# folkol/query-engines

Hardware: AMD Instinct MI355X
Metric: rows/sec filter+project+group-by over 1B-row Arrow batch; % HBM roofline (higher is better)
Workload: dtype int64; 1 GPU; C4: SELECT k, SUM(a+b), COUNT(*), MIN(a), MAX(b) WHERE a > 2^19 GROUP BY k; rows_per_gpu=1000000000, groups=1024, columns=k, a, b int64 (Arrow, no nulls), parallelism=hash-sharded partial aggregate x1

## Files before the change

### query-engines_amd/csrc/qe_jit.hip

```cpp
#include <hip/hiprtc.h>
#include <stdio.h>
#include <stdlib.h>
#include <fcntl.h>
#include <string.h>
#include <sys/stat.h>
#include <unistd.h>

#include <map>
#include <mutex>
#include <sstream>
#include <vector>

#include "qe_internal.hpp"

namespace qe {

static const char* kDevHeader =
#include "qe_dev.inc"
    ;

namespace {

struct Expr {
  std::string v;
  std::string ok;
  bool f;
};

std::string col_raw(int c) { return "c" + std::to_string(c) + "[r]"; }
std::string col_ok(const Plan& P, int c) {
  return P.cols[c].valid ? "((v" + std::to_string(c) + " >> r) & 1u)" : std::string("1u");
}
bool col_is_f(const Plan& P, int c) { return P.cols[c].kind == K_F64; }
std::string col_val(const Plan& P, int c) {
  return col_is_f(P, c) ? "bits_f64(" + col_raw(c) + ")" : col_raw(c);
}

bool agg_expr(const Plan& P, int j, Expr* out) {
  const DAgg& a = P.aggs[j];
  std::vector<Expr> st;
  for (int t = 0; t < a.ntok; ++t) {
    const DTok& k = a.tok[t];
    const std::string litref = "P.aggs[" + std::to_string(j) + "].tok[" + std::to_string(t) + "].lit";
    switch (k.op) {
      case T_COL: st.push_back({col_val(P, k.arg), col_ok(P, k.arg), col_is_f(P, k.arg)}); break;
      case T_LIT:
        st.push_back({k.lit_f64 ? "bits_f64(" + litref + ")" : litref, k.lit_null ? "0u" : "1u", k.lit_f64 != 0});
        break;
      case T_I2F0:
        if (st.empty()) return false;
        st.back() = {"((double)(" + st.back().v + "))", st.back().ok, true};
        break;
      case T_I2F1:
        if (st.size() < 2) return false;
        st[st.size() - 2] = {"((double)(" + st[st.size() - 2].v + "))", st[st.size() - 2].ok, true};
        break;
      default: {
        if (st.size() < 2) return false;
        const Expr b = st.back();
        st.pop_back();
        const Expr l = st.back();
        st.pop_back();
        Expr e;
        e.ok = "(" + l.ok + " & " + b.ok + ")";
        switch (k.op) {
          case T_ADD_I: e = {"((qi64)((qu64)(" + l.v + ") + (qu64)(" + b.v + ")))", e.ok, false}; break;
          case T_SUB_I: e = {"((qi64)((qu64)(" + l.v + ") - (qu64)(" + b.v + ")))", e.ok, false}; break;
          case T_MUL_I: e = {"((qi64)((qu64)(" + l.v + ") * (qu64)(" + b.v + ")))", e.ok, false}; break;
          case T_DIV_I:
            e = {"idiv((" + l.v + "), (" + b.v + "))", "(" + e.ok + " & (qu32)((" + b.v + ") != 0))", false};
            break;
          case T_ADD_F: e = {"((" + l.v + ") + (" + b.v + "))", e.ok, true}; break;
          case T_SUB_F: e = {"((" + l.v + ") - (" + b.v + "))", e.ok, true}; break;
          case T_MUL_F: e = {"((" + l.v + ") * (" + b.v + "))", e.ok, true}; break;
          case T_DIV_F: e = {"((" + l.v + ") / (" + b.v + "))", e.ok, true}; break;
          default: return false;
        }
        st.push_back(e);
      }
    }
  }
  if (st.size() != 1) return false;
  *out = st[0];
  if (out->f) out->v = "f64_bits(" + out->v + ")";
  return true;
}

const char* cmp_sym(int op) {
  switch (op) {
    case QE_OP_EQ: return "==";
    case QE_OP_NE: return "!=";
    case QE_OP_LT: return "<";
    case QE_OP_LE: return "<=";
    case QE_OP_GT: return ">";
    default: return ">=";
  }
}

std::string acc_init(int acc) {
  switch (acc) {
    case ACC_MIN_I:
    case ACC_MIN_F: return "0x7FFFFFFFFFFFFFFFll";
    case ACC_MAX_I:
    case ACC_MAX_F: return "EMPTY_KEY";
    default: return "0";
  }
}

bool use_nt() {
  const char* e = getenv("QE_NT");
  return !(e && e[0] == '0');
}
}

bool fused_prefetch() {
  static const bool v = [] {
    const char* e = getenv("QE_FUSED_PF");
    return e && e[0] == '1';
  }();
  return v;
}
int fused_block(int lds_log2) {
  (void)lds_log2;
  static const int env = [] {
    const char* e = getenv("QE_FUSED_BLOCK");
    const int b = e ? atoi(e) : 0;
    return (b == 256 || b == 512 || b == 1024) ? b : 0;
  }();
  return env ? env : 1024;
}

namespace {

std::string ld(const std::string& type, const std::string& ptr, bool nt = true) {
  if (nt && use_nt()) return "__builtin_nontemporal_load((const " + type + "*)(" + ptr + "))";
  return "(*(const " + type + "*)(" + ptr + "))";
}

void emit_predicate(const Plan& P, std::ostringstream& o, int rows) {
  const std::string loop = "#pragma unroll\n    for (int r = 0; r < " + std::to_string(rows) + "; ++r) ";
  if (P.mask_col >= 0) {
    o << loop << "if (!((qu32)(" << col_raw(P.mask_col) << " & 1) & " << col_ok(P, P.mask_col)
      << ")) act &= ~(1u << r);\n";
  }
  for (int t = 0; t < P.nterms; ++t) {
    const DTerm& T = P.terms[t];
    const std::string lit = "P.terms[" + std::to_string(t) + "].lit";
    std::string lhs, rhs, ok = col_ok(P, T.lhs);
    if (T.f64) {
      lhs = col_is_f(P, T.lhs) ? col_val(P, T.lhs) : "((double)" + col_raw(T.lhs) + ")";
      if (T.rhs >= 0) rhs = col_is_f(P, T.rhs) ? col_val(P, T.rhs) : "((double)" + col_raw(T.rhs) + ")";
      else rhs = "bits_f64(" + lit + ")";
    } else {
      lhs = col_raw(T.lhs);
      rhs = T.rhs >= 0 ? col_raw(T.rhs) : lit;
    }
    if (T.rhs >= 0) ok += " & " + col_ok(P, T.rhs);
    else if (T.lit_null) ok = "0u";
    o << loop << "if (!((" << lhs << ") " << cmp_sym(T.op) << " (" << rhs << ")) || !(" << ok
      << ")) act &= ~(1u << r);\n";
  }
}

unsigned pred_key_cols(const Plan& P) {
  unsigned m = 0;
  if (P.mask_col >= 0) m |= 1u << P.mask_col;
  for (int t = 0; t < P.nterms; ++t) {
    m |= 1u << P.terms[t].lhs;
    if (P.terms[t].rhs >= 0) m |= 1u << P.terms[t].rhs;
  }
  if (P.key_mode != 0)
    for (int k = 0; k < P.nkeys; ++k) m |= 1u << P.key_col[k];
  return m;
}

void emit_col_loads(const Plan& P, std::ostringstream& o, unsigned need, const std::string& pre = "c",
                    bool declare = true) {
  const std::string vpre = pre == "c" ? "v" : "p" + std::string("v");
  for (int c = 0; c < P.ncols; ++c) {
    if (!((need >> c) & 1u)) continue;
    const std::string cs = std::to_string(c);
    const std::string dst = pre + cs;
    if (declare) o << "    qi64 " << dst << "[4];\n";
    const int kind = P.cols[c].kind;
    const char* ty = kind == K_I32 ? "qi32" : kind == K_U8 ? "qu8" : kind == K_BOOL ? "qu8" : "qi64";
    o << "    {\n      const " << ty << "* p = (const " << ty << "*)P.cols[" << cs << "].p;\n";
    if (kind == K_BOOL) {
      o << "      for (int r = 0; r < 4; ++r) { const qi64 row = r0 + 128 * (r >> 1) + (r & 1);\n"
        << "        " << dst << "[r] = (full || row < P.n) ? ((p[row >> 3] >> (row & 7)) & 1) : 0; }\n";
    } else {
      o << "      if (full) {\n";
      if (kind == K_I64 || kind == K_F64) {
        o << "        const qi64x2 a = " << ld("qi64x2", "p + r0") << ", b = " << ld("qi64x2", "p + r0 + 128") << ";\n"
          << "        " << dst << "[0] = a.x; " << dst << "[1] = a.y; " << dst << "[2] = b.x; " << dst << "[3] = b.y;\n";
      } else if (kind == K_I32) {
        o << "        const qi32x2 a = " << ld("qi32x2", "p + r0") << ", b = " << ld("qi32x2", "p + r0 + 128") << ";\n"
          << "        " << dst << "[0] = a.x; " << dst << "[1] = a.y; " << dst << "[2] = b.x; " << dst << "[3] = b.y;\n";
      } else {
        o << "        const qu16 a = " << ld("qu16", "p + r0") << ", b = " << ld("qu16", "p + r0 + 128") << ";\n"
          << "        " << dst << "[0] = a & 0xFF; " << dst << "[1] = a >> 8; " << dst << "[2] = b & 0xFF; " << dst
          << "[3] = b >> 8;\n";
      }
      o << "      } else {\n"
        << "        for (int r = 0; r < 4; ++r) { const qi64 row = r0 + 128 * (r >> 1) + (r & 1);\n"
        << "          " << dst << "[r] = row < P.n ? (qi64)p[row] : 0; }\n      }\n";
    }
    o << "    }\n";
    if (P.cols[c].valid) {
      if (declare) o << "    qu32 " << vpre << cs << ";\n";
      o << "    {\n      const qu8* vb = P.cols[" << cs << "].valid;\n"
        << "      const qu32 lo = (full || r0 < P.n) ? ((qu32)(vb[r0 >> 3] >> (r0 & 7)) & 3u) : 0u;\n"
        << "      const qu32 hi = (full || r0 + 128 < P.n) ? ((qu32)(vb[(r0 + 128) >> 3] >> (r0 & 7)) & 3u) : 0u;\n"
        << "      " << vpre << cs << " = lo | (hi << 2);\n    }\n";
    }
  }
}

void emit_active_rows(const Plan& P, std::ostringstream& o, bool retry, bool skip_idle = true) {
  o << "    qu32 act = 15u;\n"
    << "    if (!full) { act = 0; for (int r = 0; r < 4; ++r) act |= (qu32)(r0 + 128 * (r >> 1) + (r & 1) < P.n) << r; }\n";
  if (retry)
    o << "    if (P.defer_in) {\n      for (int r = 0; r < 4; ++r) { const qi64 row = r0 + 128 * (r >> 1) + (r & 1);\n"
      << "        if (row < P.n && !((P.defer_in[row >> 5] >> (row & 31)) & 1)) act &= ~(1u << r); }\n    }\n";
  emit_predicate(P, o, 4);
  if (skip_idle) o << "    if (act == 0) continue;\n";
}

void emit_keys(const Plan& P, std::ostringstream& o) {
  o << "    qi64 key[4] = {0, 0, 0, 0};\n    qu32 knull = 0;\n";
  if (P.key_mode == 1) {
    const int c = P.key_col[0];
    o << "#pragma unroll\n    for (int r = 0; r < 4; ++r) {\n      qi64 k = " << col_raw(c) << ";\n";
    if (P.key_f64) o << "      if (bits_f64(k) != bits_f64(k)) k = 0x7FF8000000000000ll;\n";
    if (P.cols[c].valid)
      o << "      if (!" << col_ok(P, c) << ") { k = 0; knull |= 1u << r; }\n";
    o << "      key[r] = k;\n    }\n";
  } else if (P.key_mode == 2) {
    o << "#pragma unroll\n    for (int r = 0; r < 4; ++r) {\n      qi64 k = 0;\n";
    for (int q = 0; q < P.nkeys; ++q) {
      const int c = P.key_col[q];
      o << "      { const bool isn = !" << col_ok(P, c) << "; k |= ((isn ? 0ll : (" << col_raw(c) << " & "
        << P.key_fmask[q] << "ll)) << " << P.key_shift[q] << ") | ((qi64)isn << " << P.key_nullbit[q] << "); }\n";
    }
    o << "      key[r] = k;\n    }\n";
  }
}

void emit_lds_table(const Plan& P, std::ostringstream& o, int log2, size_t* lds_bytes) {
  const int S = 1 << log2, SS = S + 2;
  o << "  constexpr int LOG2 = " << log2 << ", S = " << S << ", SS = " << SS << ";\n"
    << "  __shared__ qi64 s_keys[SS];\n  __shared__ qu32 s_cst[SS];\n";
  size_t lds = (size_t)SS * 12;
  for (int j = 0; j < P.naggs; ++j) {
    const DAgg& a = P.aggs[j];
    if (a.share) {
      const int i = a.share - 1;
      if (a.acc != ACC_NONE) o << "  qi64* const s_acc" << j << " = s_acc" << i << ";\n";
      if (a.track_nn) o << "  qu32* const s_nn" << j << " = s_nn" << i << ";\n";
      if (acc_has_idx(a.acc)) o << "  qu64* const s_idx" << j << " = s_idx" << i << ";\n";
      continue;
    }
    if (a.acc != ACC_NONE) {
      o << "  __shared__ qi64 s_acc" << j << "[SS];\n";
      lds += 8 * SS;
    }
    if (a.track_nn) {
      o << "  __shared__ qu32 s_nn" << j << "[SS];\n";
      lds += 4 * SS;
    }
    if (acc_has_idx(a.acc)) {
      const int nw = a.acc == ACC_SUM_X ? fx_window_idx_words() : 4;
      o << "  __shared__ qu64 s_idx" << j << "[" << nw << " * SS];\n";
      lds += 8 * nw * SS;
    }
  }
  *lds_bytes = lds;
  o << "  for (int s = threadIdx.x; s < SS; s += blockDim.x) {\n    s_keys[s] = EMPTY_KEY;\n    s_cst[s] = 0;\n";
  for (int j = 0; j < P.naggs; ++j) {
    const DAgg& a = P.aggs[j];
    if (a.share) continue;
    if (a.acc != ACC_NONE) o << "    s_acc" << j << "[s] = " << acc_init(a.acc) << ";\n";
    if (a.track_nn) o << "    s_nn" << j << "[s] = 0;\n";
    if (acc_has_idx(a.acc))
      o << "    for (int k = 0; k < " << (a.acc == ACC_SUM_X ? fx_window_idx_words() : 4) << "; ++k) s_idx" << j << "[k * SS + s] = "
        << (acc_is_f64mm(a.acc) ? "~0ull" : "0ull") << ";\n";
  }
  o << "  }\n  __syncthreads();\n";
}

constexpr int FXQ_CAP = 128;

std::vector<int> fx_queue_aggs(const Plan& P) {
  std::vector<int> q;
  for (int j = 0; j < P.naggs; ++j)
    if (P.aggs[j].pkind != 0 && P.aggs[j].acc == ACC_SUM_X && !P.aggs[j].share) q.push_back(j);
  return q;
}

bool fx_queue_enabled() {
  static const bool v = [] {
    const char* e = getenv("QE_FX_QUEUE");
    return !(e && e[0] == '0');
  }();
  return v;
}

size_t fx_queue_bytes(const Plan& P, int block) {
  const size_t nq = fx_queue_aggs(P).size();
  return nq ? (size_t)(block / 64) * FXQ_CAP * (4 + 8 * nq) : 0;
}

void emit_fx_queue_decl(const Plan& P, std::ostringstream& o, int block) {
  const std::vector<int> q = fx_queue_aggs(P);
  o << "  __shared__ qu32 q_slot[" << (block / 64) * FXQ_CAP << "];\n";
  for (size_t k = 0; k < q.size(); ++k) o << "  __shared__ qi64 q_x" << k << "[" << (block / 64) * FXQ_CAP << "];\n";
  o << "  const qu32 q_base = (threadIdx.x >> 6) * " << FXQ_CAP << "u;\n  qu32 q_head = 0, q_n = 0;\n";
}

void emit_fx_queue_run(const Plan& P, std::ostringstream& o, const std::string& m) {
  const std::vector<int> q = fx_queue_aggs(P);
  const int nq = (int)q.size();
  o << "      __builtin_amdgcn_fence(__ATOMIC_ACQ_REL, \"wavefront\");\n"
    << "      if ((qu32)lane < " << m << ") {\n"
    << "        const qu32 qp = q_base + ((q_head + (qu32)lane) & " << FXQ_CAP - 1 << "u);\n"
    << "        const qu32 qe = q_slot[qp];\n        const int s = (int)(qe & 0xFFFFFFu);\n"
    << "        qi64 qx[" << nq << "];\n        qu32 rare = 0;\n";
  for (int k = 0; k < nq; ++k)
    o << "        qx[" << k << "] = ((qe >> " << 24 + k << ") & 1u) ? q_x" << k << "[qp] : 0ll;\n"
      << "        if (fx_rare(qx[" << k << "])) { rare |= 1u << " << k << "; qx[" << k << "] = 0; }\n";
  {
  o << "        qu64* wp0[" << nq << "];\n        qu64* wp1[" << nq << "];\n        qu64 lo[" << nq << "], hi[" << nq
    << "];\n        bool ng[" << nq << "], k0[" << nq << "];\n";
  for (int k = 0; k < nq; ++k) {
    const std::string j = std::to_string(q[k]), ks = std::to_string(k);
    o << "        {\n          const qu64 b = (qu64)qx[" << ks << "];\n          const int ex = (int)((b >> 52) & 0x7FF);\n"
      << "          const qu64 mm = ex ? ((b & ((1ull << 52) - 1)) | (1ull << 52)) : 0ull;\n"
      << "          const int p = ex ? ex - FXW_EX_LO : 0, kk = p >> 6, qq = p & 63;\n"
      << "          qu64 l = mm << qq, h = qq ? (mm >> (64 - qq)) : 0ull;\n"
      << "          ng[" << ks << "] = ex && (b >> 63);  // (-0.0 adds nothing, like +0.0)\n"
      << "          if (ng[" << ks << "]) { l = 0ull - l; h = ~h + (l == 0 ? 1ull : 0ull); }\n"
      << "          lo[" << ks << "] = l; hi[" << ks << "] = h; k0[" << ks << "] = kk == 0;\n"
      << "          wp0[" << ks << "] = kk ? &s_idx" << j << "[s] : (qu64*)&s_acc" << j << "[s];\n"
      << "          wp1[" << ks << "] = &s_idx" << j << "[kk * SS + s];\n        }\n";
  }
  o << "        qu64 o0[" << nq << "], t[" << nq << "], o1[" << nq << "];\n";
  for (int k = 0; k < nq; ++k) o << "        o0[" << k << "] = atomicAdd(wp0[" << k << "], lo[" << k << "]);\n";
  for (int k = 0; k < nq; ++k)
    o << "        t[" << k << "] = hi[" << k << "] + (o0[" << k << "] + lo[" << k << "] < o0[" << k << "] ? 1ull : 0ull);\n";
  for (int k = 0; k < nq; ++k) o << "        o1[" << k << "] = atomicAdd(wp1[" << k << "], t[" << k << "]);\n";
  for (int k = 0; k < nq; ++k) {
    const std::string j = std::to_string(q[k]), ks = std::to_string(k);
    o << "        if (k0[" << ks << "]) {\n          const qi64 d = (qi64)((t[" << ks << "] < hi[" << ks << "] ? 1 : 0) + (o1[" << ks
      << "] + t[" << ks << "] < o1[" << ks << "] ? 1 : 0)) - (ng[" << ks << "] ? 1 : 0);\n"
      << "          if (d) atomicAdd(&s_idx" << j << "[SS + s], (qu64)d);\n        }\n";
  }
  }
  o << "        if (rare) {\n          const bool knl = s == S;\n"
    << "          const qi64 key = knl ? 0 : (s == S + 1 ? EMPTY_KEY : s_keys[s]);\n";
  for (int k = 0; k < nq; ++k) {
    unsigned jm = 1u << q[k];
// ... 203 lines not shown
    << "      const qu32 kk = (qu32)key[r];\n"
    << "      const int hs = bucket2_hit(q[r], q2[r], kk, h[r], h2[r]);\n"
    << "      slot[r] = ((knull >> r) & 1) ? S : ((qi32)kk == EMPTY_KEY32 ? S + 1 : hs);\n"
    << "    }\n"
    << "    qu32 miss = 0;\n"
    << "#pragma unroll\n    for (int r = 0; r < 4; ++r) miss |= (qu32)(slot[r] < 0) << r;\n"
    << "    miss &= act & fit;\n"
    << "    if (miss) {\n      int t0 = slot[0], t1 = slot[1], t2 = slot[2], t3 = slot[3];\n"
    << "      lds_probe4_rows(s_keys, NBK, miss, (qi32)key[0], (qi32)key[1], (qi32)key[2], (qi32)key[3], h[0], h[1], h[2], h[3], t0, t1, t2, t3);\n"
    << "      slot[0] = t0; slot[1] = t1; slot[2] = t2; slot[3] = t3;\n    }\n"
    << "    qu32 glob = ~fit;\n"
    << "#pragma unroll\n    for (int r = 0; r < 4; ++r) glob |= (qu32)(slot[r] < 0) << r;\n"
    << "    glob &= act;\n    const qu32 loc = act & ~glob;\n"
    << "    int sl[4];\n"
    << "#pragma unroll\n    for (int r = 0; r < 4; ++r) sl[r] = ((loc >> r) & 1) ? slot[r] : SINK + lane;\n"
    << "#pragma unroll\n    for (int r = 0; r < 4; ++r) atomicAdd(&s_cst[sl[r]], 1u);\n";
  for (int j = 0; j < P.naggs; ++j) {
    const DAgg& a = P.aggs[j];
    if (a.pkind == 0) continue;
    const std::string js = std::to_string(j);
    const bool a32 = compact_acc32(P, j);
    o << "#pragma unroll\n    for (int r = 0; r < 4; ++r) {\n"
      << "      const int s = (" << ok[j] << ") ? sl[r] : SINK + lane;\n"
      << "      const qi64 x = " << val[j] << ";\n";
    if (a.track_nn) o << "      atomicAdd(&s_nn" << js << "[s], 1u);\n";
    switch (a.acc) {
      case ACC_SUM_I: o << "      atomicAdd((qu64*)&s_acc" << js << "[s], (qu64)x);\n"; break;
      case ACC_MIN_I: o << "      lds_min_rf(&s_acc" << js << "[s], " << (a32 ? "(qi32)x" : "x") << ");\n"; break;
      case ACC_MAX_I: o << "      lds_max_rf(&s_acc" << js << "[s], " << (a32 ? "(qi32)x" : "x") << ");\n"; break;
      default: break;
    }
    o << "    }\n";
  }
  o << "    if (glob) {\n      for (int r = 0; r < 4; ++r) {\n        if (!((glob >> r) & 1)) continue;\n"
    << "        const qi64 lr = " << didx << ";\n        qu64 gs;\n"
    << "        if (!gtable_find(P.t, key[r], (knull >> r) & 1, gs)) {\n"
    << "          atomicOr((qu32*)&P.defer_out[lr >> 5], 1u << (lr & 31));\n"
    << "          atomicAdd(&P.t.ctl[1], 1ull);\n          continue;\n        }\n"
    << "        gadd_cstar(P.t, gs, 1);\n        const qu64 row = (qu64)(" << row << ");\n";
  for (int j = 0; j < P.naggs; ++j) {
    const DAgg& a = P.aggs[j];
    if (a.pkind == 0) continue;
    o << "        if (" << ok[j] << ") { const RowVal rv = row_partial(" << a.acc << ", " << val[j]
      << ", row); gcombine(P.t, " << a.acc << ", " << j << ", gs, rv.acc, 1, rv.i0, rv.i1, rv.i2, rv.i3, "
      << (((P.nn_skip >> j) & 1) ? "false" : "true") << "); }\n";
  }
  o << "      }\n    }\n";
}

void emit_flush_c(const Plan& P, std::ostringstream& o) {
  o << "  __syncthreads();\n"
    << "  for (int s = threadIdx.x; s < SS; s += blockDim.x) {\n"
    << "    const qu32 c = s_cst[s];\n    if (c == 0) continue;\n"
    << "    const bool knl = s == S;\n    const qi64 key = knl ? 0 : (s == S + 1 ? (qi64)EMPTY_KEY32 : (qi64)s_keys[s]);\n"
    << "    qu64 gs;\n"
    << "    const bool ok = gtable_find_wg(P.t, key, knl, gs, &s_newg);\n"
    << "    qu8* rec = nullptr;\n"
    << "    if (ok) {\n      gadd_cstar(P.t, gs, c);\n    } else {\n"
    << "      const qu64 ri = atomicAdd(&P.t.ctl[2], 1ull);\n"
    << "      if (ri >= P.ovf_cap) { atomicAdd(&P.t.ctl[3], 1ull); continue; }\n"
    << "      rec = P.ovf + ri * (qu64)P.rec_bytes;\n      write_record_head(rec, key, knl, c);\n    }\n";
  int off = 24;
  for (int j = 0; j < P.naggs; ++j) {
    const DAgg& a = P.aggs[j];
    const std::string js = std::to_string(j);
    o << "    {\n      const qi64 acc = " << (a.acc != ACC_NONE ? "(qi64)s_acc" + js + "[s]" : std::string("0")) << ";\n"
      << "      const qu64 nn = " << (a.track_nn ? "s_nn" + js + "[s]" : std::string("c")) << ";\n";
    const bool skip_nn = (P.nn_skip >> j) & 1;
    if (a.fn != QE_AGG_COUNT_STAR && !(a.acc == ACC_NONE && skip_nn))
      o << "      if (ok) gcombine(P.t, " << a.acc << ", " << j << ", gs, acc, nn, ~0ull, ~0ull, ~0ull, ~0ull, "
        << (skip_nn ? "false" : "true") << ");\n";
    o << "      if (!ok) { qu64* f = (qu64*)(rec + " << off << "); f[0] = (qu64)acc; f[1] = nn; }\n    }\n";
    off += agg_rec_bytes(a.acc);
  }
  o << "  }\n";
}

}

bool agg_inputs(const Plan& P, std::vector<Expr>* ex) {
  ex->assign(P.naggs, Expr{"0", "1u", false});
  for (int j = 0; j < P.naggs; ++j)
    if (P.aggs[j].pkind != 0 && !agg_expr(P, j, &(*ex)[j])) return false;
  return true;
}

}

void emit_record_words(const Plan& P, const PartLayout& L, const std::vector<Expr>& ex, const std::string& dst,
                       std::ostringstream& o);
static void emit_fit_check(const PartLayout& L, const std::string& w, std::ostringstream& o);

bool compact_acc32(const Plan& P, int j) {
  const DAgg& a = P.aggs[j];
  if (a.acc != ACC_MIN_I && a.acc != ACC_MAX_I) return false;
  if (a.ntok != 1 || a.tok[0].op != T_COL) return false;
  const int k = P.cols[a.tok[0].arg].kind;
  return k == K_I64 || k == K_I32 || k == K_U8 || k == K_BOOL;
}

bool compact_ok(const Plan& P) {
  if (P.key_f64 || P.key_mode == 0) return false;
  for (int j = 0; j < P.naggs; ++j) {
    const int acc = P.aggs[j].acc;
    if (acc != ACC_NONE && acc != ACC_SUM_I && acc != ACC_MIN_I && acc != ACC_MAX_I) return false;
  }
  return true;
}

size_t compact_slot_bytes(const Plan& P) {
  size_t b = 8;
  for (int j = 0; j < P.naggs; ++j) {
    if (P.aggs[j].acc != ACC_NONE) b += compact_acc32(P, j) ? 4 : 8;
    if (P.aggs[j].track_nn) b += 4;
  }
  return b;
}

bool gen_fused_source(const Plan& P, int log2, std::string* src, size_t* lds_bytes, bool spill) {
  if (log2 < 4 || log2 > 16 || P.ncols < 1 || P.ncols > QE_MAX_COLS) return false;
  if (spill && P.mp_n < 2) return false;
  const bool compact = P.lds_compact > 0;
  if (compact && !compact_ok(P)) return false;
  std::vector<Expr> ex;
  if (!agg_inputs(P, &ex)) return false;
  std::vector<std::string> val(P.naggs), ok(P.naggs);
  for (int j = 0; j < P.naggs; ++j) {
    val[j] = ex[j].v;
    ok[j] = ex[j].ok;
  }
  std::ostringstream o;
  const bool pf = fused_prefetch();
  o << "\nusing namespace qe;\n"
    << "extern \"C\" __global__ void __launch_bounds__(" << fused_block(log2) << ") qe_fused(const Plan P) {\n"
    << "  __shared__ qu32 s_newg;\n  if (threadIdx.x == 0) s_newg = 0;\n";
  const int SB = spill ? P.mp_n - 1 : 0;
  if (spill && (SB & (SB - 1))) return false;
  if (spill)
    o << "  constexpr int SB = " << SB << ";\n  qi64 sp_cid[SB];\n  qu32 sp_fill[SB];\n"
      << "#pragma unroll\n  for (int b = 0; b < SB; ++b) { sp_cid[b] = -1; sp_fill[b] = 0; }\n  qu32 nfit = 0;\n";
  if (compact) emit_lds_table_c(P, o, lds_bytes);
  else emit_lds_table(P, o, log2, lds_bytes);
  const int block = fused_block(log2);
  const bool fxq = !compact && !spill && P.mp_n <= 1 && fx_queue_enabled() && !fx_queue_aggs(P).empty() &&
                   fx_queue_aggs(P).size() <= 8 && (1 << log2) + 2 < (1 << 24) &&
                   *lds_bytes + fx_queue_bytes(P, block) <= (size_t)152 * 1024;
  if (fxq) {
    emit_fx_queue_decl(P, o, block);
    *lds_bytes += fx_queue_bytes(P, block);
  }
  o << "  const int lane = threadIdx.x & 63;\n"
    << "  const qi64 wave = (blockIdx.x * (qi64)blockDim.x + threadIdx.x) >> 6;\n"
    << "  const qi64 stride = (((qi64)gridDim.x * blockDim.x) >> 6) * 256;\n";
  if (pf) {
    o << "  {\n    const qi64 base = wave * 256;\n    const bool full = base + 256 <= P.n;\n"
      << "    const qi64 r0 = base + 2 * lane;\n";
    emit_col_loads(P, o, ~0u, "p", true);
    o << "  for (qi64 base = wave * 256; base < P.n; base += stride) {\n"
      << "    const bool full = base + 256 <= P.n;\n"
      << "    const qi64 r0 = base + 2 * lane;\n";
    for (int c = 0; c < P.ncols; ++c) {
      o << "    qi64 c" << c << "[4] = {p" << c << "[0], p" << c << "[1], p" << c << "[2], p" << c << "[3]};\n";
      if (P.cols[c].valid) o << "    const qu32 v" << c << " = pv" << c << ";\n";
    }
    o << "    if (base + stride < P.n) {\n      const qi64 nb = base + stride;\n"
      << "      const bool full = nb + 256 <= P.n;\n      const qi64 r0 = nb + 2 * lane;\n";
    emit_col_loads(P, o, ~0u, "p", false);
    o << "    }\n    do {\n";
  } else {
    o << "  for (qi64 base = wave * 256; base < P.n; base += stride) {\n"
      << "    const bool full = base + 256 <= P.n;\n"
      << "    const qi64 r0 = base + 2 * lane;\n";
    emit_col_loads(P, o, ~0u);
  }
  emit_active_rows(P, o, true, !fxq && !spill);
  emit_keys(P, o);
  if (spill) {
    const PartLayout L = part_layout(P);
    const int RB = L.bytes();
    const int wb = L.narrow ? 4 : 8;
    std::vector<std::pair<int, int>> pieces;
    for (int q = 0; q < L.words;) {
      const int left = (L.words - q) * wb;
      const int n = (left >= 16 ? 16 : left >= 12 && L.narrow ? 12 : left >= 8 ? 8 : 4) / wb;
      pieces.push_back({q, n});
      q += n;
    }
    auto piece_store = [&](int q, int n) {
      const int bytes = n * wb;
      o << "            {\n";
      if (bytes == 4) {
        o << "              __builtin_amdgcn_raw_buffer_store_b32((qu32)w[" << q << "], cb, off, " << q * wb << ", 0);\n";
      } else {
        const int d = bytes / 4;
        o << "              qu32x" << d << " v;\n";
        for (int i = 0; i < n; ++i)
          if (L.narrow)
            o << "              v[" << i << "] = (qu32)w[" << q + i << "];\n";
          else
            o << "              v[" << 2 * i << "] = (qu32)w[" << q + i << "]; v[" << 2 * i + 1 << "] = (qu32)((qu64)w[" << q + i
              << "] >> 32);\n";
        o << "              __builtin_amdgcn_raw_buffer_store_b" << bytes * 8 << "(v, cb, off, " << q * wb << ", 0);\n";
      }
      o << "            }\n";
    };
    o << "    qu32 sp = 0, sbk[4] = {0, 0, 0, 0};\n"
      << "#pragma unroll\n    for (int r = 0; r < 4; ++r) {\n"
      << "      const qu32 hs = spill_hash((qu64)key[r]);\n"
      << "      if (((act >> r) & 1) && hs >= P.mp_keep) sp |= 1u << r;\n"
      << "      sbk[r] = hs & (qu32)(SB - 1);\n    }\n"
      << "    act &= ~sp;\n"
      << "#pragma unroll\n    for (int b = 0; b < SB; ++b) {\n      qu64 bal[4];\n      qu32 tot = 0;\n"
      << "#pragma unroll\n      for (int r = 0; r < 4; ++r) { bal[r] = __ballot(((sp >> r) & 1u) && sbk[r] == (qu32)b); tot += (qu32)__popcll(bal[r]); }\n"
      << "      const qu32 room = sp_cid[b] >= 0 ? (qu32)PART_CH - sp_fill[b] : 0u;\n"
      << "      if (tot && tot <= room) {\n"
      << "        const __amdgpu_buffer_rsrc_t cb = __builtin_amdgcn_make_buffer_rsrc((void*)(P.part_rec + sp_cid[b] * (PART_CH * "
      << RB << "ll)), (short)0, (int)(PART_CH * " << RB << "), 0x00020000);\n"
      << "        qu32 kb = 0;\n"
      << "#pragma unroll\n        for (int r = 0; r < 4; ++r) {\n"
      << "          if ((bal[r] >> lane) & 1) {\n"
      << "            const qu32 k = __builtin_amdgcn_mbcnt_hi((qu32)(bal[r] >> 32), __builtin_amdgcn_mbcnt_lo((qu32)bal[r], kb));\n"
      << "            const int off = (int)((sp_fill[b] + k) * " << RB << "u);\n"
      << "            qi64 w[" << L.words << "];\n";
    emit_record_words(P, L, ex, "w", o);
    emit_fit_check(L, "w", o);
    for (const auto& pc : pieces) piece_store(pc.first, pc.second);
    o << "          }\n          kb += (qu32)__popcll(bal[r]);\n        }\n"
      << "        sp_fill[b] += tot;\n"
      << "      } else if (tot) {\n"
      << "        const int leader = __ffsll((long long)__ballot(1)) - 1;\n"
      << "        qi64 id = 0;\n"
      << "        if (lane == leader) {\n"
      << "          if (sp_cid[b] >= 0) P.part_chunk[1 + sp_cid[b]] = ((qi64)b << 32) | PART_CH;\n"
      << "          id = (qi64)atomicAdd((qu64*)P.part_chunk, 1ull);\n"
      << "        }\n"
      << "        id = __shfl(id, leader);\n"
      << "        const qi64 nid = (qi64)(((qu64)__builtin_amdgcn_readfirstlane((qu32)((qu64)id >> 32)) << 32) |\n"
      << "                                (qu64)__builtin_amdgcn_readfirstlane((qu32)id));\n"
      << "        qu32 kb = 0;\n"
      << "#pragma unroll\n        for (int r = 0; r < 4; ++r) {\n"
      << "          if ((bal[r] >> lane) & 1) {\n"
      << "            const qu32 k = kb + (qu32)__popcll(bal[r] & ((1ull << lane) - 1));\n"
      << "            const qu64 pos = k < room ? (qu64)sp_cid[b] * PART_CH + sp_fill[b] + k : (qu64)nid * PART_CH + (k - room);\n"
      << "            qi64 w[" << L.words << "];\n";
    emit_record_words(P, L, ex, "w", o);
    emit_fit_check(L, "w", o);
    const char* wt = L.narrow ? "qi32" : "qi64";
    o << "            " << wt << "* const dst = (" << wt << "*)(P.part_rec + pos * " << RB << "ull);\n";
    for (int q = 0; q < L.words; ++q) o << "            dst[" << q << "] = (" << wt << ")w[" << q << "];\n";
    o << "          }\n          kb += (qu32)__popcll(bal[r]);\n        }\n"
      << "        sp_cid[b] = nid;\n        sp_fill[b] = tot - room;\n"
      << "      }\n    }\n"
      << "    if (act == 0) continue;\n";
  } else if (P.mp_n > 1)
    o << "#pragma unroll\n    for (int r = 0; r < 4; ++r)\n"
      << "      if (((act >> r) & 1) && (P.mp_pass < 0 ? spill_hash((qu64)key[r]) < P.mp_keep\n"
      << "                                              : (qu32)__umul64hi(fmix64((qu64)key[r]), (qu64)P.mp_n) != (qu32)P.mp_pass))\n"
      << "        act &= ~(1u << r);\n"
      << "    if (act == 0) continue;\n";
  if (compact)
    emit_agg_rows_c(P, o, val, ok, "P.row_base + r0 + 128 * (r >> 1) + (r & 1)", "r0 + 128 * (r >> 1) + (r & 1)");
  else
    emit_agg_rows(P, o, val, ok, "P.row_base + r0 + 128 * (r >> 1) + (r & 1)", "r0 + 128 * (r >> 1) + (r & 1)", fxq,
                  log2 <= 8);
  o << (pf ? "    } while (0);\n  }\n  }\n" : "  }\n");
  if (fxq) {
    o << "  if (q_n) {\n";
    emit_fx_queue_run(P, o, "q_n");
    o << "  }\n";
  }
  if (spill)
    o << "#pragma unroll\n  for (int b = 0; b < SB; ++b)\n"
      << "    if ((threadIdx.x & 63) == 0 && sp_cid[b] >= 0) P.part_chunk[1 + sp_cid[b]] = ((qi64)b << 32) | (qi64)sp_fill[b];\n"
      << "  if (nfit) atomicOr(&P.t.ctl[7], 1ull);\n";
  if (compact) emit_flush_c(P, o);
  else emit_flush(P, o);
  o << "  __syncthreads();\n  if (threadIdx.x == 0 && s_newg) atomicAdd(&P.t.ctl[0], (qu64)s_newg);\n}\n";
  static const bool fx_inline = [] {
    const char* e = getenv("QE_FX_INLINE");
    return !(e && e[0] == '0');
  }();
  *src = std::string(fx_inline ? "#define QE_FX_INLINE 1\n" : "") + kDevHeader + o.str();
  return true;
}

PartLayout part_layout(const Plan& P) {
  PartLayout L{};
  bool knull = false, vnull = false, cnull = false;
  for (int k = 0; k < P.nkeys; ++k) knull = knull || P.cols[P.key_col[k]].valid != nullptr;
  int nv = 0;
  unsigned cm = 0;
  for (int j = 0; j < P.naggs; ++j) {
    if (P.aggs[j].pkind == 0) continue;
    ++nv;
    vnull = vnull || P.aggs[j].track_nn;
    L.row = L.row || acc_is_f64mm(P.aggs[j].acc);
    for (int t = 0; t < P.aggs[j].ntok; ++t)
      if (P.aggs[j].tok[t].op == T_COL) cm |= 1u << P.aggs[j].tok[t].arg;
  }
  for (int c = 0; c < P.ncols; ++c)
    if ((cm >> c) & 1u) cnull = cnull || P.cols[c].valid != nullptr;
  const int wv = 1 + nv + ((knull || vnull) ? 1 : 0);
  const int wc = 1 + __builtin_popcount(cm) + ((knull || cnull) ? 1 : 0);
  L.colmode = wc < wv;
  int w = 1;
  for (int j = 0; j < P.naggs; ++j) L.val_word[j] = (!L.colmode && P.aggs[j].pkind != 0) ? w++ : -1;
  for (int c = 0; c < QE_MAX_COLS; ++c) L.col_word[c] = (L.colmode && ((cm >> c) & 1u)) ? w++ : -1;
  L.flags_word = (knull || (L.colmode ? cnull : vnull)) ? w++ : -1;
  L.row_word = L.row ? w++ : -1;
  L.words = w;
  if (P.part_narrow && !L.row && !P.key_f64) {
    bool ok = true;
    for (int c = 0; c < P.ncols; ++c)
      if (L.col_word[c] >= 0 && P.cols[c].kind == K_F64) ok = false;
    for (int j = 0; j < P.naggs; ++j)
      if (L.val_word[j] >= 0 && P.aggs[j].acc != ACC_SUM_I && P.aggs[j].acc != ACC_MIN_I && P.aggs[j].acc != ACC_MAX_I)
        ok = false;
    L.narrow = ok;
  }
  return L;
}

static void emit_fit_check(const PartLayout& L, const std::string& w, std::ostringstream& o) {
  if (!L.narrow) return;
  for (int q = 0; q < L.words; ++q)
    o << "      nfit |= (qu32)((qu64)" << w << "[" << q << "] >> 32) ^ (qu32)((qi32)" << w << "[" << q << "] >> 31);\n";
}

static std::string narrow_chunk(const std::string& w, int G, const std::string& q) {
  if (G == 1) return "(qu32)" + w + "[" + q + "]";
  return "((qu64)(qu32)" + w + "[2 * (" + q + ")] | ((qu64)(qu32)" + w + "[2 * (" + q + ") + 1] << 32))";
}

void emit_record_words(const Plan& P, const PartLayout& L, const std::vector<Expr>& ex, const std::string& dst,
                       std::ostringstream& o) {
  o << "      " << dst << "[0] = key[r];\n";
  for (int j = 0; j < P.naggs; ++j)
    if (L.val_word[j] >= 0) o << "      " << dst << "[" << L.val_word[j] << "] = " << ex[j].v << ";\n";
  for (int c = 0; c < P.ncols; ++c)
    if (L.col_word[c] >= 0) o << "      " << dst << "[" << L.col_word[c] << "] = " << col_raw(c) << ";\n";
  if (L.flags_word >= 0) {
    o << "      " << dst << "[" << L.flags_word << "] = (qi64)((knull >> r) & 1)";
    for (int j = 0; j < P.naggs; ++j)
      if (L.val_word[j] >= 0) o << " | ((qi64)((" << ex[j].ok << ") & 1u) << " << (1 + j) << ")";
    for (int c = 0; c < P.ncols; ++c)
      if (L.col_word[c] >= 0 && P.cols[c].valid) o << " | ((qi64)" << col_ok(P, c) << " << " << (1 + c) << ")";
    o << ";\n";
  }
  if (L.row_word >= 0)
    o << "      " << dst << "[" << L.row_word << "] = P.row_base + r0 + 128 * (r >> 1) + (r & 1);\n";
}

bool gen_part_source(const Plan& P, int log2p, bool scatter, std::string* src) {
  if (P.ncols < 1 || P.ncols > QE_MAX_COLS || log2p < 1 || log2p > 13) return false;
  std::vector<Expr> ex;
  if (!agg_inputs(P, &ex)) return false;
  const PartLayout L = part_layout(P);
  unsigned need = pred_key_cols(P);
  if (scatter) need = ~0u;
  std::ostringstream o;
  o << "\nusing namespace qe;\n"
    << "extern \"C\" __global__ void __launch_bounds__(512) " << (scatter ? "qe_pscatter" : "qe_pcount")
    << "(const Plan P) {\n"
    << "  constexpr int LOG2P = " << log2p << ", NP = 1 << LOG2P;\n";
  if (scatter)
    o << "  __shared__ qu64 s_cur[NP];\n"
      << "  for (int b = threadIdx.x; b < NP; b += blockDim.x) s_cur[b] = (qu64)P.part_off[(qi64)b * gridDim.x + blockIdx.x];\n";
  else
    o << "  __shared__ qu32 s_cnt[NP];\n"
      << "  for (int b = threadIdx.x; b < NP; b += blockDim.x) s_cnt[b] = 0;\n";
  o << "  __syncthreads();\n"
    << "  const int lane = threadIdx.x & 63;\n"
    << "  qu32 nfit = 0;\n"
    << "  const qi64 lo = (qi64)blockIdx.x * P.part_tw;\n"
    << "  const qi64 hi = lo + P.part_tw < P.n ? lo + P.part_tw : P.n;\n"
    << "  for (qi64 base = lo + (qi64)(threadIdx.x >> 6) * 256; base < hi; base += (qi64)(blockDim.x >> 6) * 256) {\n"
    << "    const bool full = base + 256 <= P.n;\n"
    << "    const qi64 r0 = base + 2 * lane;\n";
  emit_col_loads(P, o, need);
  emit_active_rows(P, o, false);
  emit_keys(P, o);
  o << "#pragma unroll\n    for (int r = 0; r < 4; ++r) {\n"
    << "      if (!((act >> r) & 1)) continue;\n"
    << "      const qu32 b = (qu32)(fmix64((qu64)key[r]) >> (64 - LOG2P));\n";
  if (!scatter) {
    o << "      atomicAdd(&s_cnt[b], 1u);\n    }\n  }\n  __syncthreads();\n"
      << "  for (int b = threadIdx.x; b < NP; b += blockDim.x) P.part_off[(qi64)b * gridDim.x + blockIdx.x] = s_cnt[b];\n}\n";
  } else {
    o << "      const qu64 pos = atomicAdd(&s_cur[b], 1ull);\n"
      << "      qi64 w[" << L.words << "];\n";
    emit_record_words(P, L, ex, "w", o);
    emit_fit_check(L, "w", o);
    if (L.narrow) {
      const int G = L.words % 2 ? 1 : 2;
      const char* ct = G == 2 ? "qu64" : "qu32";
      o << "      " << ct << "* dst = (" << ct << "*)(P.part_rec + pos * " << L.bytes() << "ull);\n";
      for (int q = 0; q < L.words / G; ++q)
        o << "      dst[" << q << "] = " << narrow_chunk("w", G, std::to_string(q)) << ";\n";
    } else if (L.words % 2 == 0) {
      o << "      qi64x2* dst = (qi64x2*)(P.part_rec + pos * " << 8 * L.words << "ull);\n";
      for (int q = 0; q < L.words / 2; ++q)
        o << "      dst[" << q << "] = qi64x2{w[" << 2 * q << "], w[" << 2 * q + 1 << "]};\n";
    } else {
      o << "      qi64* dst = (qi64*)(P.part_rec + pos * " << 8 * L.words << "ull);\n";
      for (int q = 0; q < L.words; ++q) o << "      dst[" << q << "] = w[" << q << "];\n";
    }
    o << "    }\n  }\n";
    if (L.narrow) o << "  if (nfit) atomicOr(&P.t.ctl[7], 1ull);\n";
    o << "}\n";
  }
  *src = std::string(kDevHeader) + o.str();
  return true;
}

bool part_staged_ok(const Plan& P, int log2p) {
  if (P.n < 2) return false;
  if (log2p == 10) return pscatter_wide() && part_layout(P).words <= 3;
  return log2p <= 9 && part_layout(P).words * pscatter_block() <= 8 * 256;
// ... 1669 lines not shown
```

Measured before the change: 285.3 billion rows/s.

## Split main scan loop into full-tile and tail paths with compile-time full flag

Restructures the JIT-emitted scan loop so full 256-row tiles run in a loop where `full` is a constexpr true, and the partial tail runs once afterwards. This removes per-iteration bounds checks and branches in the hot path. The prefetch path is rewritten to match. It also adds environment-gated experiment modes (QE_EXP) that insert s_waitcnt barriers or unroll two tiles per iteration. These modes are probes and are off by default.

```diff
diff --git a/query-engines_amd/csrc/qe_jit.hip b/query-engines_amd/csrc/qe_jit.hip
--- a/query-engines_amd/csrc/qe_jit.hip
+++ b/query-engines_amd/csrc/qe_jit.hip
@@ -174,9 +174,10 @@
   return m;
 }
 
+static int g_exp = 0;
 void emit_col_loads(const Plan& P, std::ostringstream& o, unsigned need, const std::string& pre = "c",
                     bool declare = true) {
-  const std::string vpre = pre == "c" ? "v" : "p" + std::string("v");
+  const std::string vpre = pre == "c" ? "v" : pre + "v";
   for (int c = 0; c < P.ncols; ++c) {
     if (!((need >> c) & 1u)) continue;
     const std::string cs = std::to_string(c);
@@ -191,7 +192,12 @@
     } else {
       o << "      if (full) {\n";
       if (kind == K_I64 || kind == K_F64) {
-        o << "        const qi64x2 a = " << ld("qi64x2", "p + r0") << ", b = " << ld("qi64x2", "p + r0 + 128") << ";\n"
+        if (g_exp == 4)
+          o << "        const qi64x2 a = " << ld("qi64x2", "p + r0") << ";\n        asm volatile(\"s_waitcnt vmcnt(0)\" ::: \"memory\");\n"
+            << "        const qi64x2 b = " << ld("qi64x2", "p + r0 + 128") << ";\n";
+        else
+        o << "        const qi64x2 a = " << ld("qi64x2", "p + r0") << ", b = " << ld("qi64x2", "p + r0 + 128") << ";\n";
+        o
           << "        " << dst << "[0] = a.x; " << dst << "[1] = a.y; " << dst << "[2] = b.x; " << dst << "[3] = b.y;\n";
       } else if (kind == K_I32) {
         o << "        const qi32x2 a = " << ld("qi32x2", "p + r0") << ", b = " << ld("qi32x2", "p + r0 + 128") << ";\n"
@@ -206,6 +212,8 @@
         << "          " << dst << "[r] = row < P.n ? (qi64)p[row] : 0; }\n      }\n";
     }
     o << "    }\n";
+    if ((g_exp == 1 && c == 0) || (g_exp == 3 && c + 1 < P.ncols) || (g_exp == 4 && c + 1 < P.ncols) || (g_exp == 5 && c == 1))
+      o << "    if (full) asm volatile(\"s_waitcnt vmcnt(0)\" ::: \"memory\");\n";
     if (P.cols[c].valid) {
       if (declare) o << "    qu32 " << vpre << cs << ";\n";
       o << "    {\n      const qu8* vb = P.cols[" << cs << "].valid;\n"
@@ -715,27 +723,7 @@
   o << "  const int lane = threadIdx.x & 63;\n"
     << "  const qi64 wave = (blockIdx.x * (qi64)blockDim.x + threadIdx.x) >> 6;\n"
     << "  const qi64 stride = (((qi64)gridDim.x * blockDim.x) >> 6) * 256;\n";
-  if (pf) {
-    o << "  {\n    const qi64 base = wave * 256;\n    const bool full = base + 256 <= P.n;\n"
-      << "    const qi64 r0 = base + 2 * lane;\n";
-    emit_col_loads(P, o, ~0u, "p", true);
-    o << "  for (qi64 base = wave * 256; base < P.n; base += stride) {\n"
-      << "    const bool full = base + 256 <= P.n;\n"
-      << "    const qi64 r0 = base + 2 * lane;\n";
-    for (int c = 0; c < P.ncols; ++c) {
-      o << "    qi64 c" << c << "[4] = {p" << c << "[0], p" << c << "[1], p" << c << "[2], p" << c << "[3]};\n";
-      if (P.cols[c].valid) o << "    const qu32 v" << c << " = pv" << c << ";\n";
-    }
-    o << "    if (base + stride < P.n) {\n      const qi64 nb = base + stride;\n"
-      << "      const bool full = nb + 256 <= P.n;\n      const qi64 r0 = nb + 2 * lane;\n";
-    emit_col_loads(P, o, ~0u, "p", false);
-    o << "    }\n    do {\n";
-  } else {
-    o << "  for (qi64 base = wave * 256; base < P.n; base += stride) {\n"
-      << "    const bool full = base + 256 <= P.n;\n"
-      << "    const qi64 r0 = base + 2 * lane;\n";
-    emit_col_loads(P, o, ~0u);
-  }
+  const auto emit_step = [&]() {
   emit_active_rows(P, o, true, !fxq && !spill);
   emit_keys(P, o);
   if (spill) {
@@ -826,7 +814,103 @@
   else
     emit_agg_rows(P, o, val, ok, "P.row_base + r0 + 128 * (r >> 1) + (r & 1)", "r0 + 128 * (r >> 1) + (r & 1)", fxq,
                   log2 <= 8);
-  o << (pf ? "    } while (0);\n  }\n  }\n" : "  }\n");
+  };
+  const auto step_head = [&](bool full, const char* base) {
+    o << "    constexpr bool full = " << (full ? "true" : "false") << ";\n    const qi64 r0 = " << base << " + 2 * lane;\n";
+  };
+  g_exp = getenv("QE_EXP") ? atoi(getenv("QE_EXP")) : 0;
+  if (g_exp == 2 || g_exp == 7) {
+    o << "  qi64 base = wave * 512;\n";
+    o << "  for (; base + 512 <= P.n; base += 2 * stride) {\n    constexpr bool full = true;\n";
+    for (const char* pre : {"p", "q"})
+      for (int c = 0; c < P.ncols; ++c) {
+        o << "    qi64 " << pre << c << "[4];\n";
+        if (P.cols[c].valid) o << "    qu32 " << pre << "v" << c << ";\n";
+      }
+    if (g_exp == 7) {
+      for (int c = 0; c < P.ncols; ++c) {
+        o << "    {\n    const qi64 r0 = base + 2 * lane;\n";
+        emit_col_loads(P, o, 1u << c, "p", false);
+        o << "    }\n    {\n    const qi64 r0 = base + 256 + 2 * lane;\n";
+        emit_col_loads(P, o, 1u << c, "q", false);
+        o << "    }\n";
+        if (c + 1 < P.ncols) o << "    asm volatile(\"s_waitcnt vmcnt(0)\" ::: \"memory\");\n";
+      }
+    } else {
+    o << "    {\n    const qi64 r0 = base + 2 * lane;\n";
+    emit_col_loads(P, o, ~0u, "p", false);
+    o << "    }\n    {\n    const qi64 r0 = base + 256 + 2 * lane;\n";
+    emit_col_loads(P, o, ~0u, "q", false);
+    o << "    }\n";
+    }
+    for (int t = 0; t < 2; ++t) {
+      const char* pre = t ? "q" : "p";
+      o << "    {\n    const qi64 r0 = base + " << 256 * t << " + 2 * lane;\n";
+      for (int c = 0; c < P.ncols; ++c) {
+        o << "    qi64 c" << c << "[4] = {" << pre << c << "[0], " << pre << c << "[1], " << pre << c << "[2], " << pre << c << "[3]};\n";
+        if (P.cols[c].valid) o << "    const qu32 v" << c << " = " << pre << "v" << c << ";\n";
+      }
+      o << "    do {\n";
+      emit_step();
+      o << "    } while (0);\n    }\n";
+    }
+    o << "  }\n";
+    o << "  if (base + 256 <= P.n) {\n";
+    step_head(true, "base");
+    emit_col_loads(P, o, ~0u);
+    o << "    do {\n";
+    emit_step();
+    o << "    } while (0);\n    base += 256;\n  }\n";
+    o << "  if (base < P.n) do {\n";
+    step_head(false, "base");
+    emit_col_loads(P, o, ~0u);
+    emit_step();
+    o << "  } while (0);\n";
+  } else {
+  o << "  qi64 base = wave * 256;\n";
+  if (pf) {
+    o << "  {\n";
+    for (int c = 0; c < P.ncols; ++c) {
+      o << "  qi64 p" << c << "[4] = {0, 0, 0, 0};\n";
+      if (P.cols[c].valid) o << "  qu32 pv" << c << " = 0;\n";
+    }
+    const auto emit_next_loads = [&](const char* nb) {
+      o << "    if (" << nb << " + 256 <= P.n) {\n";
+      step_head(true, nb);
+      emit_col_loads(P, o, ~0u, "p", false);
+      o << "    } else if (" << nb << " < P.n) {\n";
+      step_head(false, nb);
+      emit_col_loads(P, o, ~0u, "p", false);
+      o << "    }\n";
+    };
+    emit_next_loads("base");
+    for (int full = 1; full >= 0; --full) {
+      o << (full ? "  for (; base + 256 <= P.n; base += stride) {\n" : "  if (base < P.n) {\n");
+      step_head(full, "base");
+      for (int c = 0; c < P.ncols; ++c) {
+        o << "    qi64 c" << c << "[4] = {p" << c << "[0], p" << c << "[1], p" << c << "[2], p" << c << "[3]};\n";
+        if (P.cols[c].valid) o << "    const qu32 v" << c << " = pv" << c << ";\n";
+      }
+      if (full) {
+        o << "    {\n    const qi64 nb = base + stride;\n";
+        emit_next_loads("nb");
+        o << "    }\n";
+      }
+      o << "    do {\n";
+      emit_step();
+      o << "    } while (0);\n  }\n";
+    }
+    o << "  }\n";
+  } else {
+    for (int full = 1; full >= 0; --full) {
+      o << (full ? "  for (; base + 256 <= P.n; base += stride) {\n" : "  if (base < P.n) do {\n");
+      step_head(full, "base");
+      emit_col_loads(P, o, ~0u);
+      emit_step();
+      o << (full ? "  }\n" : "  } while (0);\n");
+    }
+  }
+  }
   if (fxq) {
     o << "  if (q_n) {\n";
     emit_fx_queue_run(P, o, "q_n");
```

Measured after the change: 270.9 billion rows/s. 5.0% lower.
